# pangenome/smoothxg

Hardware: AMD Instinct MI355X
Metric: POA blocks/sec (+ DP cells/sec) on 1000-block synthetic (higher is better)
Workload: dtype int16

## Files before the change

### smoothxg_amd/csrc/poa_graph_dev.h

```cpp
#pragma once
#include "poa_types.h"

namespace sxg {


template <class Ctx, class F, class P>
SXG_HD int array_excl_sum(Ctx& c, int n, F get, P out) {
    constexpr int SCAN_K = Ctx::SCAN_K;
    const int T = c.nthreads(), t = c.tid();
    int carry = 0;
    for (int base = 0; base < n; base += SCAN_K * T) {
        const int i0 = base + SCAN_K * t;
        int v[SCAN_K], s = 0;
#pragma unroll
        for (int k = 0; k < SCAN_K; ++k) v[k] = i0 + k < n ? get(i0 + k) : 0;
#pragma unroll
        for (int k = 0; k < SCAN_K; ++k) s += v[k];
        int tot;
        int p = carry + c.scan_excl_add(s, &tot);
#pragma unroll
        for (int k = 0; k < SCAN_K; ++k) {
            if (i0 + k < n) out[i0 + k] = p;
            p += v[k];
        }
// ... 523 lines not shown
    }
    array_excl_sum(c, n, [&](int s) { return cnt[s]; }, cnt);
    c.sync();
    SXG_RSP(2);
    if (!full) {
        for (int x0 = t; x0 < n; x0 += GB * T) {
            int s[GB], rk[GB], wk[GB], b0[GB], p0[GB];
#pragma unroll
            for (int u = 0; u < GB; ++u) { const int x = x0 + u * T < n ? x0 + u * T : n - 1; s[u] = (int)W[x] & SPOA_FMASK; rk[u] = G.sp_rank[x]; }
#pragma unroll
            for (int u = 0; u < GB; ++u) { wk[u] = walk[s[u]]; b0[u] = cnt[s[u]]; p0[u] = pmin[s[u]]; }
#pragma unroll
            for (int u = 0; u < GB; ++u) { const int x = x0 + u * T; if (x < n && !wk[u]) G.order[b0[u] + rk[u] - p0[u]] = x; }
        }
    }
    {
        SXG_GP const SpoaHalf* const rh = (SXG_GP const SpoaHalf*)rec;
        const int nw = sdem[n + 2];
        for (int k = t; k < nw; k += T) {
            const int v = list[k];
            const SpoaHalf ra = rh[4 * (size_t)v], rb = rh[4 * (size_t)v + 1];
            const int ob = cnt[v], sb = sdem[v];
            spoa_walk_root(G, W, v, G.order + ob, G.dfs_stack + c.atomic_add((int32_t*)(sdem + n), sb), ra, rb);
        }
    }
    c.sync();
    SXG_RSP(3);
    for (int r0 = t; r0 < n; r0 += GB * T) {
        int v[GB];
#pragma unroll
        for (int u = 0; u < GB; ++u) v[u] = r0 + u * T < n ? G.order[r0 + u * T] : 0;
#pragma unroll
        for (int u = 0; u < GB; ++u) { const int r = r0 + u * T; if (r < n) { G.rank[v[u]] = r; G.sp_rank[v[u]] = r; } }
    }
    for (int x = t; x < n; x += T) G.sp_first[x] = (int)W[x] & SPOA_FMASK;
    SXG_RSP(4);
}

template <class Ctx, class LdsP>
SXG_HD_PHASE void spoa_resort(Ctx& c, const GraphView& G_, LdsP lst, const int lst_cap, const int n_static, const int len, const int n_prev,
                              const bool full, unsigned long long* rprof = nullptr) {
    const GraphView G = sxg_scalar_view(G_);
    const int n = *G.n_nodes;
    const int ns = n_static < n ? (n_static > 0 ? n_static : 0) : n;
    if (lst_cap >= 4 * (n + 1)) spoa_resort_par(c, G, sxg_as_i32(lst), n, ns, len, n_prev, full, rprof);
    else spoa_resort_par(c, G, G.newidx, n, ns, len, n_prev, full, rprof);
}

struct RowCaps {
    int rows_cap;
    int pool_slots;
    int step_cap;
    int lds_rows;
};

template <class Ctx>
SXG_HD_PHASE int finish_rows(Ctx& c, int N, const RowsView& R, const RowCaps& caps, const int hinted = 0) {
    const int T = c.nthreads(), t = c.tid();
    c.sync();
    const int n_store = array_excl_sum(c, N, [&](int r) { return (R.flags[r] & ROW_STORE) ? 1 : 0; }, R.sseq);
    if (t == 0) R.sseq[N] = n_store;
    c.sync();
    constexpr int GB = Ctx::GB;
    int worst = 0;
    for (int r0 = t; r0 < N; r0 += GB * T) {
        int fl[GB], lu[GB], sr[GB], sl[GB];
#pragma unroll
        for (int u = 0; u < GB; ++u) {
            const int r = r0 + u * T;
            fl[u] = r < N ? (int)R.flags[r] : 0;
            lu[u] = r < N ? R.slot[r] : 0;
            sr[u] = r < N ? R.sseq[r] : 0;
        }
#pragma unroll
        for (int u = 0; u < GB; ++u) sl[u] = (fl[u] & ROW_STORE) ? R.sseq[lu[u]] : 0;
#pragma unroll
        for (int u = 0; u < GB; ++u) {
            const int r = r0 + u * T;
            if (r >= N) continue;
            if (!(fl[u] & ROW_STORE)) { R.slot[r] = -1; continue; }
            const int cnt = sl[u] - sr[u];
            if (cnt > worst) worst = cnt;
            if (hinted == 1 && caps.lds_rows > 0 && cnt <= caps.lds_rows) R.slot[r] = -2 - sr[u] % caps.lds_rows;
            else R.slot[r] = sr[u] % caps.pool_slots;
        }
    }
    worst = c.reduce_max(worst);
    if (worst > caps.pool_slots && hinted < 2) return ST_POOL_OVERFLOW;
    if (!hinted) {
        const int n_steps = array_excl_sum(c, N, [&](int r) {
            const int d = R.pred_off[r + 1] - R.pred_off[r];
            return d > 1 ? d - 1 : 0; }, R.tbx);
        c.sync();
        if (n_steps > caps.step_cap) return ST_TBX_OVERFLOW;
        for (int r = t; r < N; r += T)
            if (R.pred_off[r + 1] - R.pred_off[r] <= 1) R.tbx[r] = -1;
        c.sync();
    }
    constexpr int GBH = Ctx::GBH;
    for (int r0 = t; r0 < N; r0 += GBH * T) {
        int pb[GBH], np[GBH], cf[GBH], p0[GBH], p1[GBH], q0[GBH], q1[GBH], ms[GBH], mt[GBH];
#pragma unroll
        for (int u = 0; u < GBH; ++u) {
            const int r = r0 + u * T;
            pb[u] = r < N ? R.pred_off[r] : 0;
            np[u] = r < N ? R.pred_off[r + 1] - pb[u] : 0;
            cf[u] = r < N ? ((int)R.code[r] << 16) | ((int)R.flags[r] << 24) : 0;
            ms[u] = r < N ? R.slot[r] : 0;
            mt[u] = r < N ? R.tbx[r] : 0;
        }
#pragma unroll
        for (int u = 0; u < GBH; ++u) {
            p0[u] = np[u] >= 1 ? R.preds[pb[u]] : 0;
            p1[u] = np[u] >= 2 ? R.preds[pb[u] + 1] : 0;
        }
#pragma unroll
        for (int u = 0; u < GBH; ++u) {
            const int r = r0 + u * T;
            if (hinted == 3) { q0[u] = 0; q1[u] = 0; }
            else if (hinted == 2) {
                q0[u] = p0[u] >= 1 ? R.tbx[p0[u] - 1] : 0;
                q1[u] = p1[u] >= 1 ? R.tbx[p1[u] - 1] : 0;
            } else {
                q0[u] = (p0[u] >= 1 && p0[u] != r) ? R.slot[p0[u] - 1] : -1;
                q1[u] = (p1[u] >= 1 && p1[u] != r) ? R.slot[p1[u] - 1] : -1;
            }
        }
#pragma unroll
        for (int u = 0; u < GBH; ++u) {
            const int r = r0 + u * T;
            if (r >= N) continue;
            int32_t* d = R.meta + 8 * (size_t)r;
            d[0] = pb[u]; d[1] = np[u] | cf[u]; d[2] = p0[u]; d[3] = q0[u]; d[4] = p1[u]; d[5] = q1[u]; d[6] = ms[u]; d[7] = mt[u];
        }
    }
    c.sync();
    return ST_OK;
}

template <class Ctx>
SXG_HD_PHASE void rows_remain(Ctx& c, const GraphView& G, int N, SXG_GP int32_t* out) {
    const int T = c.nthreads(), t = c.tid();
    SXG_GP int32_t* nx[2] = {G.preva, G.newidx};
    SXG_GP int32_t* ds[2] = {G.nexta, G.target};
    c.sync();
    constexpr int GB = Ctx::GB;
    for (int r0 = t; r0 < N; r0 += GB * T) {
        int e[GB], best[GB];
        uint32_t bw[GB];
#pragma unroll
        for (int u = 0; u < GB; ++u) { e[u] = r0 + u * T < N ? G.out_head[G.order[r0 + u * T]] : -1; best[u] = -1; bw[u] = 0; }
#pragma unroll
        for (int u = 0; u < GB; ++u)
            for (int x = e[u]; x >= 0; x = G.e_next_out[x]) {
                const uint32_t w = G.e_w[x];
                if (best[u] < 0 || w > bw[u]) { best[u] = G.e_head[x]; bw[u] = w; }
            }
#pragma unroll
        for (int u = 0; u < GB; ++u) {
            const int r = r0 + u * T;
            if (r >= N) continue;
            nx[0][r] = best[u] >= 0 ? G.rank[best[u]] : -1;
            ds[0][r] = best[u] >= 0 ? 1 : 0;
        }
    }
    c.sync();
    int cur = 0;
    for (int round = 0; round < 32; ++round) {
        int open = 0;
        for (int r0 = t; r0 < N; r0 += GB * T) {
            int n1[GB], d1[GB], n2[GB], d2[GB];
#pragma unroll
            for (int u = 0; u < GB; ++u) { const int r = r0 + u * T; n1[u] = r < N ? nx[cur][r] : -1; d1[u] = r < N ? ds[cur][r] : 0; }
#pragma unroll
            for (int u = 0; u < GB; ++u) { n2[u] = n1[u] >= 0 ? nx[cur][n1[u]] : -1; d2[u] = n1[u] >= 0 ? ds[cur][n1[u]] : 0; }
#pragma unroll
            for (int u = 0; u < GB; ++u) {
                const int r = r0 + u * T;
                if (r >= N) continue;
                nx[cur ^ 1][r] = n2[u];
                ds[cur ^ 1][r] = d1[u] + d2[u];
                open |= (int)(n2[u] >= 0);
            }
        }
        cur ^= 1;
        open = c.reduce_max(open);
        if (!open) break;
// ... 131 lines not shown
```

### smoothxg_amd/csrc/poa_kernels.hip.h

```cpp
#pragma once
#include <hip/hip_runtime.h>
#include <algorithm>
#include <cstdlib>
#include <cstring>

#include "../../include/sxg_poa.h"
#include "poa_classes.h"
#include "poa_dp.hip.h"
#include "poa_dp16.hip.h"
#include "poa_band16.hip.h"
#include "poa_graph_dev.h"
#include "poa_bgraph_dev.h"

using namespace sxg;


struct SlotLayout {
    size_t hdr, code, rank, order, order_tmp, leader, gmem, in_head, in_tail, out_head, out_tail, in_deg,
        out_deg, e_tail, e_head, e_next_in, e_next_out, e_w, posnode, target, newidx, nexta, preva, slotadd,
        kind, xpos, via, dfs_stack, dfs_rec, sp_rank, sp_first, sp_cnt, r_code, r_flags, r_pred_off, r_preds, r_slot, r_tbx, r_sseq, r_row_node, r_meta, tb, steps, pool,
        row0, park, cons_sc, cons_pr, pair_row, pair_pos, total;
    int nodes_cap, rows_cap, pool_slots, step_cap, scratch_len, Lpad, word_bytes, threads;
    int band_strips;
    int lds_rows;
    int W2, band_strips2;
};

inline size_t lay(size_t& cur, size_t bytes) {
    size_t o = cur;
    cur += (bytes + 255) & ~(size_t)255;
    return o;
}

inline SlotLayout make_layout(int nodes_cap, int rows_cap, int pool_slots, int step_cap, int threads, int Lpad,
                              int word_bytes, bool pairs, int band_strips = 0, int cell_bytes = 4, bool spoa_scratch = false,
                              int W2 = 0, int band_strips2 = 0) {
    SlotLayout L;
    memset(&L, 0, sizeof(L));
    L.nodes_cap = nodes_cap; L.rows_cap = rows_cap; L.pool_slots = pool_slots;
    L.step_cap = step_cap; L.threads = threads; L.Lpad = Lpad; L.word_bytes = word_bytes;
    L.band_strips = band_strips;
    const bool packed = band_strips > 0;
    L.W2 = packed ? W2 : 0; L.band_strips2 = L.W2 ? band_strips2 : 0;
    const size_t C = (size_t)nodes_cap + 4, S = (size_t)std::max(nodes_cap, Lpad) + 4, Rr = (size_t)rows_cap + 4;
    L.scratch_len = (int)S;
    size_t cur = 0;
    L.hdr = lay(cur, 512);
    L.code = lay(cur, C);
    L.rank = lay(cur, 4 * C); L.order = lay(cur, 4 * C); L.order_tmp = lay(cur, 4 * C); L.leader = lay(cur, 4 * C);
    L.gmem = lay(cur, 20 * C);
    L.in_head = lay(cur, 4 * C); L.in_tail = lay(cur, 4 * C); L.out_head = lay(cur, 4 * C);
    L.out_tail = lay(cur, 4 * C); L.in_deg = lay(cur, 4 * C); L.out_deg = lay(cur, 4 * C);
    L.e_tail = lay(cur, 4 * C); L.e_head = lay(cur, 4 * C); L.e_next_in = lay(cur, 4 * C);
    L.e_next_out = lay(cur, 4 * C); L.e_w = lay(cur, 4 * C);
    L.posnode = lay(cur, 4 * S); L.target = lay(cur, 4 * S); L.newidx = lay(cur, 4 * S);
    L.nexta = lay(cur, 4 * S); L.preva = lay(cur, 4 * S); L.slotadd = lay(cur, 4 * S); L.kind = lay(cur, S);
    L.xpos = lay(cur, 4 * C);
    L.via = lay(cur, 4 * C);
    L.dfs_stack = lay(cur, spoa_scratch ? 4 * (7 * C + 8) : 256);
    L.dfs_rec = lay(cur, spoa_scratch ? 64 * C : 256);
    L.sp_rank = lay(cur, spoa_scratch ? 4 * C : 256); L.sp_first = lay(cur, spoa_scratch ? 4 * C : 256); L.sp_cnt = lay(cur, spoa_scratch ? 4 * C : 256);
    L.r_code = lay(cur, Rr); L.r_flags = lay(cur, Rr); L.r_pred_off = lay(cur, 4 * Rr);
    L.r_preds = lay(cur, 4 * C); L.r_slot = lay(cur, 4 * Rr); L.r_tbx = lay(cur, 4 * Rr);
    L.r_sseq = lay(cur, 4 * Rr); L.r_row_node = lay(cur, 4 * Rr); L.r_meta = lay(cur, 32 * Rr);
    size_t plane_row = packed ? (size_t)band_strips * (size_t)p16_slot_dwords(Lpad / (2 * threads), cell_bytes) * 4 : (size_t)Lpad;
    if (L.W2) plane_row = std::max(plane_row, (size_t)L.band_strips2 * (size_t)p16_slot_dwords(L.W2, cell_bytes) * 4);
    L.tb = lay(cur, ((size_t)rows_cap + 1) * plane_row);
    L.steps = lay(cur, packed ? 256 : (size_t)std::max(step_cap, 1) * 3 * threads * 4);
    const size_t row_bytes = (size_t)Lpad * (packed && cell_bytes == 2 ? 2 : word_bytes) + (size_t)threads * 4;
    L.pool = lay(cur, (size_t)pool_slots * row_bytes);
    L.row0 = lay(cur, row_bytes);
    L.park = lay(cur, (size_t)Lpad * word_bytes);
    L.cons_sc = lay(cur, 8 * C); L.cons_pr = lay(cur, 4 * C);
    if (pairs) { L.pair_row = lay(cur, 4 * (Rr + Lpad)); L.pair_pos = lay(cur, 4 * (Rr + Lpad)); }
    L.total = cur;
    return L;
}

inline int p16_lds_rows(const int T, const int W, const int CB) {
    if (const char* e = getenv("SXG_POA_LDS_ROWS")) return std::max(0, std::min(8, atoi(e)));
    const int wg_per_cu = std::max(1, 16 / std::max(T / 64, 1));
    const int share = (160 * 1024) / wg_per_cu - 512;
    const int rows = (share - dp16_lds_bytes(T, W, 0, CB)) / dp16_row_bytes(T, W, CB);
    return std::max(0, std::min(8, rows));
}

inline int plane_strips_p16(int T, int W) {
    if (const char* e = getenv("SXG_POA_BAND_COLS")) {
        const int cols = std::max(atoi(e), W);
        return std::min(plane_round4((cols + W - 1) / W), 2 * T);
    }
    return p16_band_strips(T, W);
}

inline bool width2_enabled() {
    const char* e = getenv("SXG_POA_WIDTH2");
    return !(e && atoi(e) == 0);
}

struct P16LaunchSizes { int strips, strips2, lds_rows, smem; };
inline P16LaunchSizes p16_launch_sizes(int T, int W, int W2, int CB, bool wide_band) {
    P16LaunchSizes s;
    s.strips = wide_band ? 2 * T : plane_strips_p16(T, W);
    s.strips2 = W2 ? (wide_band ? 2 * T : plane_strips_p16(T, W2)) : 0;
    s.lds_rows = p16_lds_rows(T, W, CB);
    s.smem = std::max(dp16_lds_bytes(T, W, s.lds_rows, CB), W2 ? dp16_lds_bytes(T, W2, s.lds_rows, CB) : 0);
    return s;
}

struct SlotViews {
    GraphView G;
    RowsView R;
    DpBuffers B;
    int64_t* cons_sc;
    int32_t* cons_pr;
    int32_t *pair_row, *pair_pos;
};

__device__ static SlotViews slot_views(uint8_t* base, const SlotLayout& L) {
    SlotViews V;
    SXG_GP int32_t* hdr = (SXG_GP int32_t*)(base + L.hdr);
    V.G.n_nodes = hdr; V.G.n_edges = hdr + 1;
    V.G.code = (SXG_GP uint8_t*)(base + L.code);
#define P32(f) (SXG_GP int32_t*)(base + L.f)
    V.G.rank = P32(rank); V.G.order = P32(order); V.G.order_tmp = P32(order_tmp); V.G.leader = P32(leader);
    V.G.gmem = P32(gmem); V.G.in_head = P32(in_head); V.G.in_tail = P32(in_tail); V.G.out_head = P32(out_head);
    V.G.out_tail = P32(out_tail); V.G.in_deg = P32(in_deg); V.G.out_deg = P32(out_deg);
    V.G.e_tail = P32(e_tail); V.G.e_head = P32(e_head); V.G.e_next_in = P32(e_next_in);
    V.G.e_next_out = P32(e_next_out); V.G.e_w = (SXG_GP uint32_t*)(base + L.e_w);
    V.G.posnode = P32(posnode); V.G.target = P32(target); V.G.newidx = P32(newidx); V.G.nexta = P32(nexta);
    V.G.preva = P32(preva); V.G.slotadd = P32(slotadd); V.G.kind = (SXG_GP int8_t*)(base + L.kind);
    V.G.xpos = P32(xpos); V.G.via = P32(via); V.G.dfs_stack = P32(dfs_stack); V.G.dfs_rec = P32(dfs_rec);
    V.G.sp_rank = P32(sp_rank); V.G.sp_first = P32(sp_first); V.G.sp_cnt = P32(sp_cnt);
    V.R.code = (SXG_GP uint8_t*)(base + L.r_code); V.R.flags = (SXG_GP uint8_t*)(base + L.r_flags); V.R.pred_off = P32(r_pred_off);
    V.R.preds = P32(r_preds); V.R.slot = P32(r_slot); V.R.tbx = P32(r_tbx); V.R.sseq = P32(r_sseq);
    V.R.row_node = P32(r_row_node); V.R.meta = P32(r_meta);
    V.B.tb = base + L.tb; V.B.steps = (uint32_t*)(base + L.steps);
    V.B.pool = base + L.pool; V.B.row0 = base + L.row0; V.B.park = base + L.park;
    V.B.band_strips = L.band_strips; V.B.lds_rows = L.lds_rows;
// ... 2 lines not shown
#undef P32
    return V;
}

__host__ __device__ static inline Scoring normalise(const sxg_poa_params& p) {
    Scoring S;
    S.m = p.m; S.n = p.n; S.g = p.g; S.e = p.e; S.q = p.q; S.c = p.c;
    S.sw = (p.mode & 1) == SXG_MODE_LOCAL;
    S.convex = 0;
    if (S.g >= S.e) { S.e = S.g; S.q = S.g; S.c = S.g; }
    else if (S.g <= S.q || S.e >= S.c) { S.q = S.g; S.c = S.e; }
    else S.convex = 1;
    return S;
}

struct BlockArgs {
    const int32_t* blk_off; const int64_t* seq_off; const uint8_t* bases; const uint32_t* weights;
    const sxg_poa_params* params; int per_block_params;
    const int32_t* work; int n_work; int32_t* queue;
    uint8_t* arena; SlotLayout lay;
    int32_t* status; int32_t* n_nodes; int32_t* n_edges; int32_t* n_cons;
    uint8_t* node_code; int32_t* node_rank; int32_t* node_group;
    int32_t* edge_tail; int32_t* edge_head; uint32_t* edge_weight;
    int32_t* paths; int32_t* score; unsigned long long* cells; int32_t* cons_nodes;
    int want_consensus;
    int park_in_lds;
    int pf_off;
    int num_cu;
    uint32_t* prio_board;
    int prio_base;
    const unsigned long long* est;
    int lds_bytes;
    unsigned long long* blk_cycles;
    int band_floor, band_margin, band_full;
};

__host__ __device__ constexpr int sxg_min_waves(int TMAX, int W, int RM) { return class_traits(TMAX, W, RM, 4).min_waves; }

template <int TMAX, int W, bool CVX, int RM, bool SW, int CB = 4, bool DS = false, int W2 = 0>
__global__ __launch_bounds__(TMAX, sxg_min_waves(TMAX, W, RM)) void poa_block_kernel(const BlockArgs A) {
    static_assert(W2 == 0 || (RM == 2 && W2 < W), "a second strip width: packed sweep, narrower than the first");
    constexpr bool H16 = RM != 1;
    constexpr int CPL = RM >= 2 ? 2 * W : W;
    constexpr ClassTraits CT = class_traits(TMAX, W, RM, CB);
    const int T = (int)blockDim.x;
    extern __shared__ __attribute__((aligned(16))) char smem[];
    int* lds = (int*)smem;
    int& s_work = lds[200];
    WgCtx ctx{(sxg_lds_int*)(size_t)((unsigned)__builtin_amdgcn_groupstaticsize() + 128u * 4u)};
    const int t = threadIdx.x;
    SlotViews V = slot_views(A.arena + (size_t)blockIdx.x * A.lay.total, A.lay);
    V.B.prio_rank = (int)(blockIdx.x / (unsigned)A.num_cu + (unsigned)A.prio_base) & (PRIO_BOARD_SLOTS - 1);
    V.B.prio_board = A.prio_board ? A.prio_board + (size_t)(__smid() & (PRIO_BOARD_CUS - 1)) * PRIO_BOARD_SLOTS : nullptr;
    const RowCaps caps{A.lay.rows_cap, A.lay.pool_slots, A.lay.step_cap, A.lay.lds_rows};
    bool first = true;
    for (;;) {
        __syncthreads();
        if (t == 0) s_work = first ? (int)blockIdx.x : (int)gridDim.x + atomicAdd(A.queue, 1);
        first = false;
        __syncthreads();
        const int wi = s_work;
        if (wi >= A.n_work) break;
        const int b = A.work[wi];
        const unsigned long long est_total = A.est ? A.est[wi] : 0ull;
        unsigned long long done_cells = 0;
        const int s0 = A.blk_off[b], s1 = A.blk_off[b + 1];
        const int64_t base0 = A.seq_off[s0];
        const Scoring S = normalise(A.params[A.per_block_params ? b : 0]);
        if (t == 0) { *V.G.n_nodes = 0; *V.G.n_edges = 0; }
        __syncthreads();
        int status = ST_OK;
        unsigned long long* prof = (unsigned long long*)(A.arena + (size_t)blockIdx.x * A.lay.total + A.lay.hdr + 64);
        V.B.row_prof = prof + 28;
        if ((t & 63) == 0) {
            prof[10 + (t >> 6)] = ((unsigned long long)__smid() << 32) | (unsigned long long)__builtin_amdgcn_s_getreg(GETREG_IMMED(31, 0, HW_ID));
            if (t == 0 && prof[8] == 0) { prof[8] = (unsigned long long)wall_clock64(); prof[6] = (unsigned long long)clock64(); }
        }
        unsigned long long tc0 = clock64(), tc1;
        const unsigned long long tblk0 = tc0;
        int band_drift = 0, band_min = 0;
#define PROF(k) do { if (t == 0) { tc1 = clock64(); prof[k] += tc1 - tc0; tc0 = tc1; } } while (0)
        for (int s = s0; s < s1 && status == ST_OK; ++s) {
            const int64_t so = A.seq_off[s];
            const int len = (int)(A.seq_off[s + 1] - so);
            const uint8_t* seq = A.bases + so;
            for (int i = t; i < len; i += T) V.G.posnode[i] = -1;
            __syncthreads();
            const int N = *V.G.n_nodes;
            int score = 0;
            if (RM != 3 && len + 1 > T * CPL) { status = ST_TOO_LONG; break; }
            if (N + len > A.lay.nodes_cap || *V.G.n_edges + len > A.lay.nodes_cap) { status = ST_NODES_OVERFLOW; break; }
            if (RM != 1 && RM != 2 && !S.sw &&
                -(sxg_gap_cost(S.g, S.e, S.q, S.c, N) + sxg_gap_cost(S.g, S.e, S.q, S.c, len)) >= (RM >= 2 ? 15800 : 30000)) {
                status = ST_RANGE_OVERFLOW;
                break;
            }
            if (N > 0 && len > 0) {
                PROF(0);
                const int band_mode = RM == 3 ? (int)A.params[A.per_block_params ? b : 0].banded : 0;
                const int hinted_ = RM == 3 ? (band_mode == 2 ? 3 : 2) : (RM == 2 ? 1 : 0);
                if (CT.graph_batch == 16 || (CT.graph_batch == 8 && T <= 64)) { WgCtxT<16> c16{ctx.lds}; status = prep_rows(c16, V.G, V.R, caps, hinted_); }
                else if (CT.graph_batch == 8) { WgCtxT<8> c8{ctx.lds}; status = prep_rows(c8, V.G, V.R, caps, hinted_); }
                else status = prep_rows(ctx, V.G, V.R, caps, hinted_);
                if (status != ST_OK) break;
                PROF(1);
                DpResult res;
                V.B.prio_rem0 = est_total > done_cells ? est_total - done_cells : 0ull;
// ... 91 lines not shown
        }
        PROF(0);
        __syncthreads();
        const int N = *V.G.n_nodes, E = *V.G.n_edges;
        if (status == ST_OK) {
            for (int v = t; v < N; v += T) {
                A.node_code[base0 + v] = V.G.code[v];
                A.node_rank[base0 + v] = V.G.rank[v];
                A.node_group[base0 + v] = V.G.leader[v];
            }
            for (int e = t; e < E; e += T) {
                A.edge_tail[base0 + e] = V.G.e_tail[e];
                A.edge_head[base0 + e] = V.G.e_head[e];
                A.edge_weight[base0 + e] = V.G.e_w[e];
            }
            int nc = 0;
            if (A.want_consensus && t == 0) nc = consensus_serial(V.G, V.cons_sc, V.cons_pr, A.cons_nodes + base0);
            if (t == 0) { A.n_nodes[b] = N; A.n_edges[b] = E; A.n_cons[b] = nc; }
        } else if (t == 0) { A.n_nodes[b] = 0; A.n_edges[b] = 0; A.n_cons[b] = 0; }
        if (t == 0) { A.status[b] = status; if (A.blk_cycles) A.blk_cycles[b] = (unsigned long long)clock64() - tblk0; }
        if (t == 0 && V.B.prio_board) __hip_atomic_store(V.B.prio_board + V.B.prio_rank, 0u, __ATOMIC_RELAXED, __HIP_MEMORY_SCOPE_AGENT);
        PROF(5);
        if (t == 0) { prof[9] = (unsigned long long)wall_clock64(); prof[7] = (unsigned long long)clock64(); }
#undef PROF
    }
}

struct AlignArgs {
    const int64_t* row_off; const uint8_t* row_code; const uint8_t* row_sink; const int64_t* pred_off;
    const int32_t* preds; const int64_t* seq_off; const uint8_t* bases; const sxg_poa_params* params;
    int per_problem_params;
    const int32_t* work; int n_work; int32_t* queue;
    uint8_t* arena; SlotLayout lay;
    int32_t* status; int32_t* score; int32_t* n_pairs;
    int32_t* pair_row; int32_t* pair_pos;
    int park_in_lds;
    int pf_off;
    int num_cu;
};

template <int TMAX, int W, bool CVX, int RM, bool SW>
__global__ __launch_bounds__(TMAX, sxg_min_waves(TMAX, W, RM)) void poa_align_kernel(const AlignArgs A) {
    constexpr bool H16 = RM != 1;
    constexpr int CPL = RM == 2 ? 2 * W : W;
    const int T = (int)blockDim.x;
    extern __shared__ __attribute__((aligned(16))) char smem[];
    int* lds = (int*)smem;
    int& s_work = lds[200];
    WgCtx ctx{(sxg_lds_int*)(size_t)((unsigned)__builtin_amdgcn_groupstaticsize() + 128u * 4u)};
    const int t = threadIdx.x;
    SlotViews V = slot_views(A.arena + (size_t)blockIdx.x * A.lay.total, A.lay);
    V.B.prio_rank = (int)(blockIdx.x / (unsigned)A.num_cu) & (PRIO_BOARD_SLOTS - 1);
    V.B.prio_board = nullptr; V.B.prio_rem0 = 0; V.B.row_prof = nullptr;
    const RowCaps caps{A.lay.rows_cap, A.lay.pool_slots, A.lay.step_cap, A.lay.lds_rows};
    for (;;) {
        __syncthreads();
        if (t == 0) s_work = atomicAdd(A.queue, 1);
        __syncthreads();
        const int wi = s_work;
        if (wi >= A.n_work) break;
        const int p = A.work[wi];
        const int64_t r0 = A.row_off[p];
        const int N = (int)(A.row_off[p + 1] - r0);
        const int64_t so = A.seq_off[p];
        const int len = (int)(A.seq_off[p + 1] - so);
        const Scoring S = normalise(A.params[A.per_problem_params ? p : 0]);
        const int64_t e0 = A.pred_off[r0];
        int status = ST_OK, score = 0, npairs = 0;
        if (len + 1 > T * CPL) status = ST_TOO_LONG;
        else if (N > A.lay.rows_cap) status = ST_ROWS_OVERFLOW;
        else if (N > 0 && len > 0) {
            for (int r = t; r < N; r += T) {
                V.R.code[r] = A.row_code[r0 + r];
                V.R.pred_off[r] = (int)(A.pred_off[r0 + r] - e0);
                V.R.row_node[r] = r;
                V.R.slot[r] = r;
                V.R.tbx[r] = 0;
                int fl = A.row_sink[r0 + r] ? ROW_SINK : 0;
                for (int64_t k = A.pred_off[r0 + r]; k < A.pred_off[r0 + r + 1]; ++k)
                    if (A.preds[k] == r) fl |= ROW_REGPRED;
                V.R.flags[r] = (uint8_t)fl;
            }
            if (t == 0) V.R.pred_off[N] = (int)(A.pred_off[r0 + N] - e0);
            __syncthreads();
            const int E = V.R.pred_off[N];
            for (int k = t; k < E; k += T) V.R.preds[k] = A.preds[e0 + k];
            __syncthreads();
            for (int r = t; r < N; r += T)
                for (int k = V.R.pred_off[r]; k < V.R.pred_off[r + 1]; ++k) {
                    const int pr = V.R.preds[k];
                    if (pr >= 1 && pr != r) {
                        atomicOr((unsigned*)(V.R.flags + ((pr - 1) & ~3)), (unsigned)ROW_STORE << (8 * ((pr - 1) & 3)));
                        atomicMax(&V.R.slot[pr - 1], r);
                    }
                }
            status = finish_rows(ctx, N, V.R, caps, RM == 2 ? 1 : 0);
            if (status == ST_OK) {
                DpResult res;
                if constexpr (RM == 2) res = dp_fill_p16<W, CVX, SW, 4>(S, V.R, N, A.bases + so, len, V.B, smem);
                else dp_fill<W, CVX, H16, SW>(S, V.R, N, A.bases + so, len, V.B, smem, A.park_in_lds != 0, A.pf_off, res);
                __syncthreads();
                if constexpr (RM == 2) {
                    if (t == 0) { lds[TBM_FLAG] = 0; lds[TBM_RANGE] = 0; }
                    __syncthreads();
                    if (t < 64 && res.bi >= 0) npairs = traceback_p16<true, W, CVX, false, 4, true>(V.R, V.B, S, A.bases + so, len, res.best, T, min(256, (len << 8) / max(N, 1)), res.bi, res.bj, nullptr, V.pair_row, V.pair_pos, smem);
                    __syncthreads();
                    if (lds[TBM_FLAG]) status = ST_BAND_MISS;
// ... 16 lines not shown
```

### smoothxg_amd/csrc/sxg_poa.hip

```cpp
#include <hip/hip_runtime.h>
#include <algorithm>
#include <chrono>
#include <cmath>
#include <cstdio>
#include <cstdlib>
#include <cstring>
#include <memory>
#include <new>
#include <string>
#include <sys/mman.h>
#include <thread>
#include <vector>

#include "../../include/sxg_poa.h"
#include <rccl/rccl.h>
#include <dlfcn.h>
#include "poa_kernels.hip.h"
#include "poa_kern_tables.hip.h"
#include "poa_split.hip.h"
#include "poa_mash.hip.h"
#include "poa_identity.hip.h"
#include "poa_sgd.hip.h"


// ... 540 lines not shown
        if (k >= 2) A.band_margin = std::max(m, 0);
        if (k >= 3) A.band_full = std::max(n, 0);
    }
}

static void prepare_plan(sxg_poa_handle* h, LaunchPlan& P, int attempt) {
    const Variant V = P.variant;
    const int Lpad = V.Lpad();
    int nodes_cap = 0, maxlen = 0;
    bool any_adaptive = false;
    bool any_spoa = false;
    double rows_est = 0;
    for (int b : P.work) {
        const BlockMeta& m = h->meta[b];
        any_adaptive = any_adaptive || h->h_params[h->per_block_params ? b : 0].banded == 2;
        any_spoa = any_spoa || (h->h_params[h->per_block_params ? b : 0].mode & SXG_ORDER_SPOA) != 0;
        nodes_cap = (int)std::max<int64_t>(nodes_cap, m.sumlen);
        maxlen = std::max(maxlen, m.maxlen);
        rows_est = std::max(rows_est, (double)m.maxlen * std::max(2.0, 1.0 + 0.0165 * m.nseq));
    }
    nodes_cap += 8;
    const int nodes_full = nodes_cap;
    int rows_cap, pool_slots, step_cap;
    if (attempt == 0) {
        rows_cap = (int)std::min<double>(nodes_cap, rows_est + 1024);
        pool_slots = std::min(rows_cap + 1, 768);
        step_cap = rows_cap;
        nodes_cap = (int)std::min<int64_t>(nodes_full, 2LL * rows_cap + maxlen + 8);
    } else if (attempt == 1) {
        rows_cap = (int)std::min<double>(nodes_cap, 2.5 * rows_est + 4096);
        pool_slots = std::min(rows_cap + 1, 4096);
        step_cap = 3 * rows_cap;
        nodes_cap = (int)std::min<int64_t>(nodes_full, 2LL * rows_cap + maxlen + 8);
    } else if (attempt == 2) {
        rows_cap = nodes_cap; pool_slots = std::min(rows_cap + 1, 32768); step_cap = nodes_cap;
    } else {
        rows_cap = nodes_cap; pool_slots = rows_cap + 1; step_cap = nodes_cap;
    }
    if (rows_cap >= (1 << 20)) rows_cap = (1 << 20) - 1;
    const int wb = V.RM == 1 ? 8 : 4;
    if (V.RM == 3) pool_slots = 1;
    const int strips1 = V.RM == 3 ? (any_adaptive ? BAND_WIN : band_plane_strips(maxlen, V.W)) : (V.RM == 2 ? p16_launch_sizes(V.T(), V.W, 0, V.CB, P.wide_band).strips : 0);
    P.variant.TMAX = class_tmax(V.W, V.NW, V.RM, V.CB, strips1 == 2 * V.T());
    P.variant.W2 = width2_enabled() ? class_w2(CLASS_BLOCK, P.variant, P.sw) : 0;
    const P16LaunchSizes LS = p16_launch_sizes(V.T(), V.W, P.variant.W2, V.CB, P.wide_band);
    P.lay = make_layout(nodes_cap, rows_cap, pool_slots, step_cap, V.T(), Lpad, wb, false, strips1, V.RM >= 2 ? V.CB : 4, any_spoa,
                        V.RM == 2 ? P.variant.W2 : 0, LS.strips2);
    P.kern = block_kernel(P.variant, P.cvx, P.sw);
    const int tfix = class_traits(P.variant.TMAX, V.W, V.RM, V.CB).tfix;
    if (tfix && tfix != V.T()) { P.kern = nullptr; P.why = "kernel class compiled for " + std::to_string(tfix) + " threads asked to run at " + std::to_string(V.T()); }
    if (!P.kern && P.why.empty()) P.why = "no kernel class built for this geometry";
    P.smem = dp_lds_launch_bytes(Lpad, wb);
    P.park_lds = dp_park_in_lds(Lpad, wb);
    if (V.RM == 2) { P.lay.lds_rows = LS.lds_rows; P.smem = LS.smem; P.park_lds = true; }
    if (V.RM == 3) { P.smem = band_lds_bytes(V.W); P.park_lds = true; }
    P.pf_off = (V.RM < 2 && getenv("SXG_POA_PREFETCH")) ? dp_pf_offset(Lpad, wb, V.T()) : -1;
    if (P.pf_off >= 0) P.smem += dp_pf_bytes(Lpad, wb, V.T());
    if (P.smem > 48 * 1024)
        (void)hipFuncSetAttribute((const void*)P.kern, hipFuncAttributeMaxDynamicSharedMemorySize, P.smem);
    P.per_cu = 1;
    if (hipOccupancyMaxActiveBlocksPerMultiprocessor(&P.per_cu, (const void*)P.kern, V.T(), (size_t)P.smem) != hipSuccess || P.per_cu < 1)
        P.per_cu = 1;
    P.want_slots = std::min<int64_t>((int64_t)P.work.size(), (int64_t)h->num_cu * P.per_cu);
}

static int sample_clock(const LaunchPlan& P, const PlanRes& R) {
    unsigned long long cyc = 0, ticks = 0;
    const int64_t step = std::max<int64_t>(1, P.n_slots / 24);
    for (int64_t sl = 0; sl < P.n_slots; sl += step) {
        unsigned long long v[10];
        if (hipMemcpy(v, R.arena.as<uint8_t>() + (size_t)sl * P.lay.total + P.lay.hdr + 64, sizeof(v), hipMemcpyDeviceToHost) != hipSuccess) return 0;
        if (v[9] <= v[8] || v[7] <= v[6]) continue;
        cyc += v[7] - v[6];
        ticks += v[9] - v[8];
    }
    return ticks ? (int)((double)cyc / (double)ticks * 100.0 + 0.5) : 0;
}

static int launch_plan(sxg_poa_handle* h, LaunchPlan& P, PlanRes& R, const int prio_base) {
    const Variant V = P.variant;
    int rc;
    if (!P.kern) return fail(SXG_E_INVALID, P.why);
    if ((rc = R.arena.ensure((size_t)P.n_slots * P.lay.total))) return rc;
    {
        const int64_t ns = P.n_slots, ncu = std::max(h->num_cu, 1);
        const int64_t rem = ns % ncu, full = ns / ncu;
        if (rem > 0 && full >= 1 && (int64_t)P.work.size() >= ns) {
            std::vector<int32_t> first((size_t)ns, -1);
            size_t next = 0;
            for (int64_t p = 0; p < ns; ++p)
                if (p % ncu >= rem && p / ncu < full) first[(size_t)p] = P.work[next++];
            for (int64_t round = 0; round <= full; ++round)
                for (int64_t c = 0; c < rem; ++c) {
                    const int64_t cu = (round & 1) ? rem - 1 - c : c, p = round * ncu + cu;
                    if (p < ns && first[(size_t)p] < 0) first[(size_t)p] = P.work[next++];
                }
            std::copy(first.begin(), first.end(), P.work.begin());
        }
    }
    if ((rc = R.work.ensure(4 * P.work.size())) || (rc = R.queue.ensure(256)) || (rc = R.est.ensure(8 * P.work.size()))) return rc;
    HIPCHK(hipMemcpyAsync(R.work.p, P.work.data(), 4 * P.work.size(), hipMemcpyHostToDevice, R.stream));
    P.est.resize(P.work.size());
    for (size_t k = 0; k < P.work.size(); ++k) P.est[k] = (unsigned long long)std::max(h->meta[P.work[k]].cost, 1.0);
    HIPCHK(hipMemcpyAsync(R.est.p, P.est.data(), 8 * P.est.size(), hipMemcpyHostToDevice, R.stream));
    HIPCHK(hipMemsetAsync(R.queue.p, 0, 256, R.stream));
    BlockArgs A;
    A.blk_off = h->d_blk_off.as<int32_t>(); A.seq_off = h->d_seq_off.as<int64_t>(); A.bases = h->d_bases.as<uint8_t>();
// ... 2 lines not shown
    A.work = R.work.as<int32_t>(); A.n_work = (int)P.work.size(); A.queue = R.queue.as<int32_t>();
    A.arena = R.arena.as<uint8_t>(); A.lay = P.lay;
    A.status = h->d_status.as<int32_t>(); A.n_nodes = h->d_nn.as<int32_t>(); A.n_edges = h->d_ne.as<int32_t>();
    A.n_cons = h->d_nc.as<int32_t>(); A.node_code = h->d_node_code.as<uint8_t>();
    A.node_rank = h->d_node_rank.as<int32_t>(); A.node_group = h->d_node_group.as<int32_t>();
    A.edge_tail = h->d_edge_tail.as<int32_t>(); A.edge_head = h->d_edge_head.as<int32_t>();
    A.edge_weight = h->d_edge_w.as<uint32_t>(); A.paths = h->d_paths.as<int32_t>(); A.score = h->d_score.as<int32_t>();
    A.cells = h->d_cells.as<unsigned long long>(); A.cons_nodes = h->d_cons.as<int32_t>();
    A.want_consensus = h->want_consensus;
    A.park_in_lds = P.park_lds ? 1 : 0;
    A.pf_off = P.pf_off;
    A.num_cu = std::max(h->num_cu, 1);
    A.prio_board = getenv("SXG_POA_NO_BALANCE") ? nullptr : h->d_board.as<uint32_t>();
    A.prio_base = prio_base;
    A.est = R.est.as<unsigned long long>();
    A.blk_cycles = h->d_blk_cycles.as<unsigned long long>();
    A.lds_bytes = getenv("SXG_POA_RESORT_NO_LDS") ? 0 : P.smem;
    band_adapt_args(A);
    HIPCHK(hipMemset2DAsync(R.arena.as<uint8_t>() + P.lay.hdr, P.lay.total, 0, 512, (size_t)P.n_slots, R.stream));
    HIPCHK(hipStreamWaitEvent(R.stream, h->ev0, 0));
    HIPCHK(hipEventRecord(R.e0, R.stream));
    hipLaunchKernelGGL(P.kern, dim3((unsigned)P.n_slots), dim3(V.T()), (size_t)P.smem, R.stream, A);
    HIPCHK(hipGetLastError());
    HIPCHK(hipEventRecord(R.e1, R.stream));
    HIPCHK(hipStreamWaitEvent(h->stream, R.e1, 0));
    return SXG_OK;
}

static int width_stats_of(const LaunchPlan& P, const PlanRes& R, sxg_poa_width_stats& w) {
    if (P.variant.RM != 2 || P.n_slots <= 0) return SXG_OK;
    constexpr int K0 = 27, K1 = 55;
    std::vector<unsigned long long> v((size_t)P.n_slots * (K1 - K0));
    HIPCHK(hipMemcpy2D(v.data(), (K1 - K0) * 8, R.arena.as<uint8_t>() + P.lay.hdr + 64 + K0 * 8, P.lay.total, (K1 - K0) * 8, (size_t)P.n_slots, hipMemcpyDeviceToHost));
    for (int64_t sl = 0; sl < P.n_slots; ++sl) {
        const unsigned long long* c = v.data() + (size_t)sl * (K1 - K0);
        w.hint_shift_repeats += c[27 - K0];
        for (int k = 0; k < 2; ++k) { w.sweeps[k] += c[49 + k - K0]; w.swept_cols[k] += c[51 + k - K0]; w.swept_cells[k] += c[53 + k - K0]; }
    }
    return SXG_OK;
}

static int debug_plan(sxg_poa_handle* h, LaunchPlan& P, PlanRes& R, int attempt) {
    const Variant V = P.variant;
    unsigned long long acc[8] = {0}, smin = ~0ull, smax = 0;
    for (int64_t sl = 0; sl < P.n_slots; ++sl) {
        unsigned long long one[8];
        HIPCHK(hipMemcpy(one, R.arena.as<uint8_t>() + (size_t)sl * P.lay.total + P.lay.hdr + 64, 64, hipMemcpyDeviceToHost));
        for (int k = 0; k < 8; ++k) acc[k] += one[k];
        unsigned long long st = 0;
        for (int k = 0; k < 6; ++k) st += one[k];
        smin = std::min(smin, st); smax = std::max(smax, st);
    }
    if (V.RM == 2) {
        unsigned long long rep = 0, wsum = 0, nsw = 0;
        for (int64_t sl = 0; sl < P.n_slots; ++sl) {
            unsigned long long v[49];
            HIPCHK(hipMemcpy(v, R.arena.as<uint8_t>() + (size_t)sl * P.lay.total + P.lay.hdr + 64, sizeof(v), hipMemcpyDeviceToHost));
            rep += v[27]; wsum += v[47]; nsw += v[48];
        }
        fprintf(stderr, "[sxg]   band: %llu sweeps, mean width %.1f strips of %d (%.0f columns), %llu hint-shift repeats\n", nsw,
                (double)wsum / (double)std::max(nsw, 1ull), P.lay.band_strips, (double)wsum / (double)std::max(nsw, 1ull) * V.W, rep);
        sxg_poa_width_stats w{};
        if (int rcw = width_stats_of(P, R, w)) return rcw;
        fprintf(stderr, "[sxg]   width: W=%d %llu sweeps %llu columns %.4g cells; W2=%d %llu sweeps %llu columns %.4g cells\n", V.W, (unsigned long long)w.sweeps[0],
                (unsigned long long)w.swept_cols[0], (double)w.swept_cells[0], P.lay.W2, (unsigned long long)w.sweeps[1], (unsigned long long)w.swept_cols[1], (double)w.swept_cells[1]);
    }
    if (const char* path = getenv("SXG_POA_SLOT_CSV")) {
        if (FILE* f = fopen(path, "a")) {
            for (int64_t sl = 0; sl < P.n_slots; ++sl) {
                unsigned long long v[26];
                HIPCHK(hipMemcpy(v, R.arena.as<uint8_t>() + (size_t)sl * P.lay.total + P.lay.hdr + 64, sizeof(v), hipMemcpyDeviceToHost));
                fprintf(f, "%lld,%llu,%llu", (long long)sl, v[8], v[9]);
                for (int w = 0; w < V.NW && w < 16; ++w) fprintf(f, ",%llx", v[10 + w]);
                fprintf(f, "\n");
            }
            fclose(f);
        }
    }
#ifdef SXG_ROW_PROF
    {
        unsigned long long ra[13] = {0};
        for (int64_t sl = 0; sl < P.n_slots; ++sl) {
            unsigned long long one[13];
            HIPCHK(hipMemcpy(one, R.arena.as<uint8_t>() + (size_t)sl * P.lay.total + P.lay.hdr + 64 + 28 * 8, sizeof(one), hipMemcpyDeviceToHost));
            for (int k = 0; k < 13; ++k) ra[k] += one[k];
        }
        double rt = 1e-9;
        for (int k = 0; k < 8; ++k) rt += (double)ra[k];
        static const char* seg16[8] = {"setup", "pass1+scan", "wait left wave", "combine+pass2", "wait right wave", "hand-over+end cell", "stored row fetch", "outgoing+row store"};
        static const char* segb[8] = {"descriptor+band", "predecessor fetch+fold", "pass1+scan+pass2", "end cell+best-cell search", "outgoing+band stores", "-", "-", "-"};
        const char* const* seg = V.RM == 3 ? segb : seg16;
        fprintf(stderr, "[sxg]   row profile:");
        for (int k = 0; k < 8; ++k) fprintf(stderr, " %s %.1f%%", seg[k], 100.0 * (double)ra[k] / rt);
        fprintf(stderr, "\n");
        fprintf(stderr, "[sxg]   traceback: %.3g steps, %.1f steps per window, %.0f %% of the windows prefetched, %.0f cycles per step of which %.0f in window fills\n",
                (double)ra[8], (double)ra[8] / std::max<double>((double)ra[9], 1), 100.0 * (double)ra[12] / std::max<double>((double)ra[9], 1),
                (double)ra[10] / std::max<double>((double)ra[8], 1), (double)ra[11] / std::max<double>((double)ra[8], 1));
    }
#endif
#ifdef SXG_RESORT_PROF
    {
        unsigned long long ra[6] = {0};
        for (int64_t sl = 0; sl < P.n_slots; ++sl) {
            unsigned long long one[6];
            HIPCHK(hipMemcpy(one, R.arena.as<uint8_t>() + (size_t)sl * P.lay.total + P.lay.hdr + 64 + 41 * 8, sizeof(one), hipMemcpyDeviceToHost));
            for (int k = 0; k < 6; ++k) ra[k] += one[k];
        }
        double rt = 1e-9;
        for (int k = 0; k < 5; ++k) rt += (double)ra[k];
        fprintf(stderr, "[sxg]   re-sort: records %.1f%% first() %.1f%% counts %.1f%% walks %.1f%% ranks %.1f%%; %.3g cycles per slot, %.1f rounds per slot\n",
                100 * ra[0] / rt, 100 * ra[1] / rt, 100 * ra[2] / rt, 100 * ra[3] / rt, 100 * ra[4] / rt, rt / (double)P.n_slots, (double)ra[5] / (double)P.n_slots);
    }
// ... 1253 lines not shown
    };
#define CK(x) do { int _rc = (x); if (_rc) { cleanup(); sxg_poa_align_free(out); return _rc; } } while (0)
#define HCK(x) do { hipError_t _e = (x); if (_e != hipSuccess) { cleanup(); sxg_poa_align_free(out); return fail(SXG_E_NODEVICE, std::string(#x) + ": " + hipGetErrorString(_e)); } } while (0)
    const int np = in->per_problem_params ? n : 1;
    std::vector<uint8_t> stage((size_t)std::max<int64_t>(nbases, 1));
    for (int64_t i = 0; i < nbases; ++i) stage[i] = in->bases[i] > 4 ? 4 : in->bases[i];
    std::vector<uint8_t> codes((size_t)std::max<int64_t>(rows, 1));
    for (int64_t i = 0; i < rows; ++i) codes[i] = in->row_code[i] > 4 ? 4 : in->row_code[i];
    const size_t outcap = (size_t)(rows + nbases + 1);
    CK(d_row_off.ensure(8 * (size_t)(n + 1))); CK(d_code.ensure((size_t)rows + 16)); CK(d_sink.ensure((size_t)rows + 16));
    CK(d_pred_off.ensure(8 * (size_t)(rows + 1))); CK(d_preds.ensure(4 * (size_t)(ne + 1))); CK(d_seq_off.ensure(8 * (size_t)(n + 1)));
    CK(d_bases.ensure((size_t)nbases + 16)); CK(d_params.ensure(sizeof(sxg_poa_params) * (size_t)std::max(np, 1)));
    CK(d_status.ensure(4 * (size_t)std::max(n, 1))); CK(d_score.ensure(4 * (size_t)std::max(n, 1))); CK(d_np.ensure(4 * (size_t)std::max(n, 1)));
    CK(d_pr.ensure(4 * outcap)); CK(d_pp.ensure(4 * outcap)); CK(d_work.ensure(4 * (size_t)std::max(n, 1))); CK(d_queue.ensure(256));
    if (n) {
        HCK(hipMemcpy(d_row_off.p, in->row_off, 8 * (size_t)(n + 1), hipMemcpyHostToDevice));
        HCK(hipMemcpy(d_seq_off.p, in->seq_off, 8 * (size_t)(n + 1), hipMemcpyHostToDevice));
        HCK(hipMemcpy(d_pred_off.p, in->pred_off, 8 * (size_t)(rows + 1), hipMemcpyHostToDevice));
        HCK(hipMemcpy(d_params.p, in->params, sizeof(sxg_poa_params) * (size_t)np, hipMemcpyHostToDevice));
        if (rows) {
            HCK(hipMemcpy(d_code.p, codes.data(), (size_t)rows, hipMemcpyHostToDevice));
            HCK(hipMemcpy(d_sink.p, in->row_sink, (size_t)rows, hipMemcpyHostToDevice));
        }
        if (ne) HCK(hipMemcpy(d_preds.p, in->preds, 4 * (size_t)ne, hipMemcpyHostToDevice));
        if (nbases) HCK(hipMemcpy(d_bases.p, stage.data(), (size_t)nbases, hipMemcpyHostToDevice));
        HCK(hipMemset(d_status.p, 0, 4 * (size_t)n)); HCK(hipMemset(d_score.p, 0, 4 * (size_t)n)); HCK(hipMemset(d_np.p, 0, 4 * (size_t)n));

    }
    struct APlan { Variant variant; bool cvx, sw; std::vector<int32_t> work; int rows_cap = 0; };
    std::vector<APlan> plans;
    for (int p = 0; p < n; ++p) {
        const Scoring S = normalise(in->params[in->per_problem_params ? p : 0]);
        const int len = (int)(in->seq_off[p + 1] - in->seq_off[p]), N = (int)(in->row_off[p + 1] - in->row_off[p]);
        Variant v;
        int fw, fnw;
        forced_p16(&fw, &fnw);
        if (!variant_for_len(len, row_mode(S, len, N), &v, S.sw, 4, fw, fnw)) { o->status[p] = ST_TOO_LONG; continue; }
        APlan* pl = nullptr;
        for (auto& q : plans)
            if (q.variant == v && q.cvx == (bool)S.convex && q.sw == (bool)S.sw) { pl = &q; break; }
        if (!pl) { plans.push_back(APlan{v, (bool)S.convex, (bool)S.sw, {}, 0}); pl = &plans.back(); }
        pl->work.push_back(p);
        pl->rows_cap = std::max(pl->rows_cap, N);
    }
    if (n) HCK(hipMemcpy(d_status.p, o->status.data(), 4 * (size_t)n, hipMemcpyHostToDevice));
    for (auto& pl : plans) {
        const Variant V = pl.variant;
        const int rows_cap = pl.rows_cap + 1;
        int64_t maxe = 0;
        for (int p : pl.work) maxe = std::max<int64_t>(maxe, in->pred_off[in->row_off[p + 1]] - in->pred_off[in->row_off[p]]);
        const int wb = V.RM == 1 ? 8 : 4;
        SlotLayout lay2 = make_layout((int)std::max<int64_t>(maxe + 8, rows_cap + 8), rows_cap, rows_cap + 1,
                                      (int)maxe + 8, V.T(), V.Lpad(), wb, true, V.RM == 2 ? 2 * V.T() : 0);
        if (V.RM == 2) lay2.lds_rows = p16_lds_rows(V.T(), V.W, 4);
        auto kern = align_kernel(pl.variant, pl.cvx, pl.sw);
        const int tfix = class_traits(V.TMAX, V.W, V.RM, V.CB).tfix;
        if (!kern || (tfix && tfix != V.T())) { cleanup(); sxg_poa_align_free(out); return fail(SXG_E_INVALID, kern ? "kernel class compiled for another thread count" : "no kernel class built for this geometry"); }
        int per_cu = 1;
        int smem = V.RM == 2 ? dp16_lds_bytes(V.T(), V.W, lay2.lds_rows, 4) : dp_lds_launch_bytes(V.Lpad(), wb);
        const int pf_off = (V.RM != 2 && getenv("SXG_POA_PREFETCH")) ? dp_pf_offset(V.Lpad(), wb, V.T()) : -1;
        if (pf_off >= 0) smem += dp_pf_bytes(V.Lpad(), wb, V.T());
        if (smem > 48 * 1024) (void)hipFuncSetAttribute((const void*)kern, hipFuncAttributeMaxDynamicSharedMemorySize, smem);
        if (hipOccupancyMaxActiveBlocksPerMultiprocessor(&per_cu, (const void*)kern, V.T(), (size_t)smem) != hipSuccess || per_cu < 1) per_cu = 1;
        const uint64_t budget = arena_budget(h);
        int64_t n_slots = std::min<int64_t>((int64_t)pl.work.size(), (int64_t)h->num_cu * per_cu);
        n_slots = std::min<int64_t>(n_slots, (int64_t)(budget / lay2.total));
        if (n_slots < 1) { cleanup(); sxg_poa_align_free(out); return fail(SXG_E_NOMEM, "memory budget too small for one alignment arena"); }
        CK(d_arena.ensure((size_t)n_slots * lay2.total));
        HCK(hipMemcpy(d_work.p, pl.work.data(), 4 * pl.work.size(), hipMemcpyHostToDevice));
        HCK(hipMemset(d_queue.p, 0, 4));
        AlignArgs A;
        A.row_off = d_row_off.as<int64_t>(); A.row_code = d_code.as<uint8_t>(); A.row_sink = d_sink.as<uint8_t>();
        A.pred_off = d_pred_off.as<int64_t>(); A.preds = d_preds.as<int32_t>(); A.seq_off = d_seq_off.as<int64_t>();
        A.bases = d_bases.as<uint8_t>(); A.params = d_params.as<sxg_poa_params>(); A.per_problem_params = in->per_problem_params;
        A.work = d_work.as<int32_t>(); A.n_work = (int)pl.work.size(); A.queue = d_queue.as<int32_t>();
        A.arena = d_arena.as<uint8_t>(); A.lay = lay2;
        A.status = d_status.as<int32_t>(); A.score = d_score.as<int32_t>(); A.n_pairs = d_np.as<int32_t>();
        A.pair_row = d_pr.as<int32_t>(); A.pair_pos = d_pp.as<int32_t>();
        A.park_in_lds = (V.RM == 2 || dp_park_in_lds(V.Lpad(), wb)) ? 1 : 0;
        A.pf_off = pf_off;
        A.num_cu = std::max(h->num_cu, 1);
        hipLaunchKernelGGL(kern, dim3((unsigned)n_slots), dim3(V.T()), (size_t)smem, h->stream, A);
        HCK(hipGetLastError());
        HCK(hipStreamSynchronize(h->stream));
    }
    std::vector<int32_t> npairs(std::max(n, 1), 0), pr(outcap), pp(outcap);
    if (n) {
        HCK(hipMemcpy(o->status.data(), d_status.p, 4 * (size_t)n, hipMemcpyDeviceToHost));
        HCK(hipMemcpy(o->score.data(), d_score.p, 4 * (size_t)n, hipMemcpyDeviceToHost));
        HCK(hipMemcpy(npairs.data(), d_np.p, 4 * (size_t)n, hipMemcpyDeviceToHost));
        HCK(hipMemcpy(pr.data(), d_pr.p, 4 * outcap, hipMemcpyDeviceToHost));
        HCK(hipMemcpy(pp.data(), d_pp.p, 4 * outcap, hipMemcpyDeviceToHost));
    }
    for (int p = 0; p < n; ++p) o->pair_off[p + 1] = o->pair_off[p] + npairs[p];
    o->pair_row.resize((size_t)std::max<int64_t>(o->pair_off[n], 1)); o->pair_pos.resize(o->pair_row.size());
    for (int p = 0; p < n; ++p) {
        const int64_t s0 = in->row_off[p] + in->seq_off[p];
        std::copy(pr.begin() + s0, pr.begin() + s0 + npairs[p], o->pair_row.begin() + o->pair_off[p]);
        std::copy(pp.begin() + s0, pp.begin() + s0 + npairs[p], o->pair_pos.begin() + o->pair_off[p]);
    }
    cleanup();
#undef CK
#undef HCK
    out->status = o->status.data(); out->score = o->score.data(); out->pair_off = o->pair_off.data();
    out->pair_row = o->pair_row.data(); out->pair_pos = o->pair_pos.data();
    for (int p = 0; p < n; ++p)
        if (o->status[p] != ST_OK) return fail(SXG_E_BLOCK, "problem " + std::to_string(p) + " failed with status " + std::to_string(o->status[p]));
// ... 620 lines not shown
```

Baseline: 688.5.

## Assign on-chip LDS row copies via liveness-based free list instead of FIFO

Replaces the modulo (FIFO) assignment of stored DP rows to the few LDS row buffers with a greedy interval-based free list. The free list reuses a buffer once its previous row's last consumer has passed, so more stored rows and their reads should stay on chip instead of in the global pool. This adds a prefix-max scan and a serial per-chain assignment pass in finish_rows, plus optional debug counters for on-chip row and read fractions. The old FIFO policy stays available through an environment variable.

```diff
diff --git a/smoothxg_amd/csrc/poa_graph_dev.h b/smoothxg_amd/csrc/poa_graph_dev.h
--- a/smoothxg_amd/csrc/poa_graph_dev.h
+++ b/smoothxg_amd/csrc/poa_graph_dev.h
@@ -599,7 +599,62 @@
     int pool_slots;
     int step_cap;
     int lds_rows;
+    int lds_fifo;
+    int32_t* stat_rows;
+    int32_t* stat_reads;
 };
+
+template <class Ctx>
+SXG_HD void onchip_free_list(Ctx& c, const int n_store, const int K, SXG_GP const int32_t* const cr, SXG_GP const int32_t* const clu,
+                             SXG_GP int32_t* const pm, SXG_GP int32_t* const slot) {
+    const int T = c.nthreads(), t = c.tid();
+    c.sync();
+    array_incl_max(c, n_store, [&](int u) { return clu[u]; }, pm);
+    c.sync();
+    constexpr int GB = Ctx::GB, CH = 8;
+    for (int ub = t; ub < n_store; ub += GB * T) {
+        int rs[GB], pb[GB];
+#pragma unroll
+        for (int x = 0; x < GB; ++x) {
+            const int u0 = ub + x * T;
+            rs[x] = u0 < n_store ? cr[u0] : 0;
+            pb[x] = u0 < n_store ? (u0 > 0 ? pm[u0 - 1] : 0) : 0x7fffffff;
+        }
+#pragma unroll
+        for (int x = 0; x < GB; ++x) {
+            const int u0 = ub + x * T;
+            if (pb[x] > rs[x]) continue;
+            int freed[8], live_to = 0;
+#pragma unroll
+            for (int k = 0; k < 8; ++k) freed[k] = 0;
+            bool done = false;
+            for (int u = u0; !done; u += CH) {
+                int rr[CH], ll[CH];
+#pragma unroll
+                for (int y = 0; y < CH; ++y) {
+                    rr[y] = u + y < n_store ? cr[u + y] : 0x7fffffff;
+                    ll[y] = u + y < n_store ? clu[u + y] : 0;
+                }
+#pragma unroll
+                for (int y = 0; y < CH; ++y) {
+                    if (done) continue;
+                    const int r = rr[y], lu = ll[y];
+                    if (u + y != u0 && live_to <= r) { done = true; continue; }
+                    int best = -1, bk = -1;
+#pragma unroll
+                    for (int k = 0; k < 8; ++k)
+                        if (k < K && freed[k] <= r && freed[k] > best) { best = freed[k]; bk = k; }
+                    if (bk >= 0) {
+                        slot[r] = -2 - bk;
+#pragma unroll
+                        for (int k = 0; k < 8; ++k) if (k == bk) freed[k] = lu;
+                    }
+                    if (lu > live_to) live_to = lu;
+                }
+            }
+        }
+    }
+}
 
 template <class Ctx>
 SXG_HD_PHASE int finish_rows(Ctx& c, int N, const RowsView& R, const RowCaps& caps, const int hinted = 0) {
@@ -610,6 +665,9 @@
     c.sync();
     constexpr int GB = Ctx::GB;
     int worst = 0;
+    const bool free_list = hinted == 1 && caps.lds_rows > 0 && !caps.lds_fifo;
+    SXG_GP int32_t* const cr = R.meta;
+    SXG_GP int32_t* const clu = R.meta + N;
     for (int r0 = t; r0 < N; r0 += GB * T) {
         int fl[GB], lu[GB], sr[GB], sl[GB];
 #pragma unroll
@@ -628,10 +686,12 @@
             if (!(fl[u] & ROW_STORE)) { R.slot[r] = -1; continue; }
             const int cnt = sl[u] - sr[u];
             if (cnt > worst) worst = cnt;
-            if (hinted == 1 && caps.lds_rows > 0 && cnt <= caps.lds_rows) R.slot[r] = -2 - sr[u] % caps.lds_rows;
+            if (hinted == 1 && caps.lds_rows > 0 && caps.lds_fifo && cnt <= caps.lds_rows) R.slot[r] = -2 - sr[u] % caps.lds_rows;
             else R.slot[r] = sr[u] % caps.pool_slots;
-        }
-    }
+            if (free_list) { cr[sr[u]] = r; clu[sr[u]] = lu[u]; }
+        }
+    }
+    if (free_list) onchip_free_list(c, n_store, caps.lds_rows < 8 ? caps.lds_rows : 8, cr, clu, R.meta + 2 * (size_t)N, R.slot);
     worst = c.reduce_max(worst);
     if (worst > caps.pool_slots && hinted < 2) return ST_POOL_OVERFLOW;
     if (!hinted) {
@@ -645,6 +705,8 @@
         c.sync();
     }
     constexpr int GBH = Ctx::GBH;
+    const bool count = hinted == 1 && caps.stat_rows != nullptr;
+    int n_st = 0, n_st_chip = 0, n_rd = 0, n_rd_chip = 0;
     for (int r0 = t; r0 < N; r0 += GBH * T) {
         int pb[GBH], np[GBH], cf[GBH], p0[GBH], p1[GBH], q0[GBH], q1[GBH], ms[GBH], mt[GBH];
 #pragma unroll
@@ -679,7 +741,20 @@
             if (r >= N) continue;
             int32_t* d = R.meta + 8 * (size_t)r;
             d[0] = pb[u]; d[1] = np[u] | cf[u]; d[2] = p0[u]; d[3] = q0[u]; d[4] = p1[u]; d[5] = q1[u]; d[6] = ms[u]; d[7] = mt[u];
-        }
+            if (count) {
+                n_st += (int)(ms[u] != -1); n_st_chip += (int)(ms[u] <= -2);
+                n_rd += (int)(q0[u] != -1) + (int)(q1[u] != -1); n_rd_chip += (int)(q0[u] <= -2) + (int)(q1[u] <= -2);
+                for (int k = 2; k < np[u]; ++k) {
+                    const int p = R.preds[pb[u] + k];
+                    const int q = (p >= 1 && p != r) ? R.slot[p - 1] : -1;
+                    n_rd += (int)(q != -1); n_rd_chip += (int)(q <= -2);
+                }
+            }
+        }
+    }
+    if (count) {
+        c.atomic_add(caps.stat_rows, n_st); c.atomic_add(caps.stat_rows + 1, n_st_chip);
+        c.atomic_add(caps.stat_reads, n_rd); c.atomic_add(caps.stat_reads + 1, n_rd_chip);
     }
     c.sync();
     return ST_OK;
diff --git a/smoothxg_amd/csrc/poa_kernels.hip.h b/smoothxg_amd/csrc/poa_kernels.hip.h
--- a/smoothxg_amd/csrc/poa_kernels.hip.h
+++ b/smoothxg_amd/csrc/poa_kernels.hip.h
@@ -23,6 +23,8 @@
     int nodes_cap, rows_cap, pool_slots, step_cap, scratch_len, Lpad, word_bytes, threads;
     int band_strips;
     int lds_rows;
+    int lds_fifo;
+    int lds_stats;
     int W2, band_strips2;
 };
 
@@ -85,6 +87,11 @@
     return std::max(0, std::min(8, rows));
 }
 
+inline int p16_lds_fifo() {
+    const char* e = getenv("SXG_POA_LDS_POLICY");
+    return e && strcmp(e, "fifo") == 0 ? 1 : 0;
+}
+
 inline int plane_strips_p16(int T, int W) {
     if (const char* e = getenv("SXG_POA_BAND_COLS")) {
         const int cols = std::max(atoi(e), W);
@@ -193,7 +200,9 @@
     SlotViews V = slot_views(A.arena + (size_t)blockIdx.x * A.lay.total, A.lay);
     V.B.prio_rank = (int)(blockIdx.x / (unsigned)A.num_cu + (unsigned)A.prio_base) & (PRIO_BOARD_SLOTS - 1);
     V.B.prio_board = A.prio_board ? A.prio_board + (size_t)(__smid() & (PRIO_BOARD_CUS - 1)) * PRIO_BOARD_SLOTS : nullptr;
-    const RowCaps caps{A.lay.rows_cap, A.lay.pool_slots, A.lay.step_cap, A.lay.lds_rows};
+    int32_t* const stat32 = (int32_t*)(A.arena + (size_t)blockIdx.x * A.lay.total + A.lay.hdr + 64);
+    const RowCaps caps{A.lay.rows_cap, A.lay.pool_slots, A.lay.step_cap, A.lay.lds_rows, A.lay.lds_fifo,
+                       A.lay.lds_stats ? stat32 + 2 * 26 : nullptr, A.lay.lds_stats ? stat32 + 2 * 55 : nullptr};
     bool first = true;
     for (;;) {
         __syncthreads();
@@ -391,7 +400,7 @@
     SlotViews V = slot_views(A.arena + (size_t)blockIdx.x * A.lay.total, A.lay);
     V.B.prio_rank = (int)(blockIdx.x / (unsigned)A.num_cu) & (PRIO_BOARD_SLOTS - 1);
     V.B.prio_board = nullptr; V.B.prio_rem0 = 0; V.B.row_prof = nullptr;
-    const RowCaps caps{A.lay.rows_cap, A.lay.pool_slots, A.lay.step_cap, A.lay.lds_rows};
+    const RowCaps caps{A.lay.rows_cap, A.lay.pool_slots, A.lay.step_cap, A.lay.lds_rows, A.lay.lds_fifo, nullptr, nullptr};
     for (;;) {
         __syncthreads();
         if (t == 0) s_work = atomicAdd(A.queue, 1);
diff --git a/smoothxg_amd/csrc/sxg_poa.hip b/smoothxg_amd/csrc/sxg_poa.hip
--- a/smoothxg_amd/csrc/sxg_poa.hip
+++ b/smoothxg_amd/csrc/sxg_poa.hip
@@ -616,7 +616,7 @@
     if (!P.kern && P.why.empty()) P.why = "no kernel class built for this geometry";
     P.smem = dp_lds_launch_bytes(Lpad, wb);
     P.park_lds = dp_park_in_lds(Lpad, wb);
-    if (V.RM == 2) { P.lay.lds_rows = LS.lds_rows; P.smem = LS.smem; P.park_lds = true; }
+    if (V.RM == 2) { P.lay.lds_rows = LS.lds_rows; P.lay.lds_fifo = p16_lds_fifo(); P.lay.lds_stats = getenv("SXG_POA_DEBUG") != nullptr; P.smem = LS.smem; P.park_lds = true; }
     if (V.RM == 3) { P.smem = band_lds_bytes(V.W); P.park_lds = true; }
     P.pf_off = (V.RM < 2 && getenv("SXG_POA_PREFETCH")) ? dp_pf_offset(Lpad, wb, V.T()) : -1;
     if (P.pf_off >= 0) P.smem += dp_pf_bytes(Lpad, wb, V.T());
@@ -725,12 +725,16 @@
         smin = std::min(smin, st); smax = std::max(smax, st);
     }
     if (V.RM == 2) {
-        unsigned long long rep = 0, wsum = 0, nsw = 0;
+        unsigned long long rep = 0, wsum = 0, nsw = 0, st_all = 0, st_chip = 0, rd_all = 0, rd_chip = 0;
         for (int64_t sl = 0; sl < P.n_slots; ++sl) {
-            unsigned long long v[49];
+            unsigned long long v[56];
             HIPCHK(hipMemcpy(v, R.arena.as<uint8_t>() + (size_t)sl * P.lay.total + P.lay.hdr + 64, sizeof(v), hipMemcpyDeviceToHost));
             rep += v[27]; wsum += v[47]; nsw += v[48];
-        }
+            st_all += v[26] & 0xffffffffull; st_chip += v[26] >> 32; rd_all += v[55] & 0xffffffffull; rd_chip += v[55] >> 32;
+        }
+        fprintf(stderr, "[sxg]   on chip (%d copies, %s): %.1f%% of %llu stored rows, %.1f%% of %llu stored-row reads\n", P.lay.lds_rows,
+                P.lay.lds_fifo ? "fifo" : "free list", 100.0 * (double)st_chip / (double)std::max(st_all, 1ull), st_all,
+                100.0 * (double)rd_chip / (double)std::max(rd_all, 1ull), rd_all);
         fprintf(stderr, "[sxg]   band: %llu sweeps, mean width %.1f strips of %d (%.0f columns), %llu hint-shift repeats\n", nsw,
                 (double)wsum / (double)std::max(nsw, 1ull), P.lay.band_strips, (double)wsum / (double)std::max(nsw, 1ull) * V.W, rep);
         sxg_poa_width_stats w{};
@@ -2090,7 +2094,7 @@
         const int wb = V.RM == 1 ? 8 : 4;
         SlotLayout lay2 = make_layout((int)std::max<int64_t>(maxe + 8, rows_cap + 8), rows_cap, rows_cap + 1,
                                       (int)maxe + 8, V.T(), V.Lpad(), wb, true, V.RM == 2 ? 2 * V.T() : 0);
-        if (V.RM == 2) lay2.lds_rows = p16_lds_rows(V.T(), V.W, 4);
+        if (V.RM == 2) { lay2.lds_rows = p16_lds_rows(V.T(), V.W, 4); lay2.lds_fifo = p16_lds_fifo(); }
         auto kern = align_kernel(pl.variant, pl.cvx, pl.sw);
         const int tfix = class_traits(V.TMAX, V.W, V.RM, V.CB).tfix;
         if (!kern || (tfix && tfix != V.T())) { cleanup(); sxg_poa_align_free(out); return fail(SXG_E_INVALID, kern ? "kernel class compiled for another thread count" : "no kernel class built for this geometry"); }
```

Result: no change. 693.5, median of 4 (+0.7%).
